# Belis0811/MaskUnet

Measured on AMD Instinct MI355X. Metric: 128x128 images/sec (fwd+bwd), higher is better.
Workload: dtype f16; 1 GPU; ADE20K-semantic shape 128x128, c_out=150, batch=64/GPU, 1-head MaskAttn-UNet fwd+bwd, train mode; global_batch=64, parallelism=dp1, mask_mode=fixed, loss=maskunet_amd.CrossEntropyLoss on module output, optimizer_in_step=False, hip_graph=False

## Files before the change

### maskunet_amd/csrc/elementwise.hip

```cpp
#include "common.h"
#include "../../include/maskunet_hip.h"

template <typename TS, typename TD>
__global__ __launch_bounds__(256) void transpose_kernel(const TS* __restrict__ src, long src_ld, TD* __restrict__ dst,
                                                        long dst_ld, int R, int C, int R_pad) {
    __shared__ float tile[64][65];
    const int b = blockIdx.z;
    const int r0 = blockIdx.y * 64, c0 = blockIdx.x * 64;
    const TS* s = src + (long)b * R * src_ld;
    TD* d = dst + (long)b * C * dst_ld;
    const int tx = threadIdx.x & 63, ty = threadIdx.x >> 6;
#pragma unroll 4
    for (int i = ty; i < 64; i += 4) {
        int r = r0 + i, c = c0 + tx;
        tile[i][tx] = (r < R && c < C) ? (float)s[(long)r * src_ld + c] : 0.f;
    }
    __syncthreads();
#pragma unroll 4
    for (int i = ty; i < 64; i += 4) {
        int c = c0 + i, r = r0 + tx;
        if (c < C && r < R_pad) d[(long)c * dst_ld + r] = (TD)tile[tx][i];
    }
}

// ... 63 lines not shown
    return mu_transpose_pad(src, src_dtype, src_ld, dst, dst_dtype, dst_ld, batch, R, C, R, stream);
}

template <typename T>
__global__ void prep_weight_kernel(const float* __restrict__ w, T* __restrict__ dst, int O, int I, int taps,
                                   int rows_pad, int cols_pad, int mode) {
    const long n = (long)taps * rows_pad * cols_pad;
    const long total = mode == 2 ? 2 * n : n;
    for (long idx = (long)blockIdx.x * blockDim.x + threadIdx.x; idx < total; idx += (long)gridDim.x * blockDim.x) {
        const bool second = idx >= n;
        const int m = mode == 2 ? (second ? 1 : 0) : mode;
        const long j = second ? idx - n : idx;
        const int rp = second ? cols_pad : rows_pad, cp = second ? rows_pad : cols_pad;
        int c = j % cp;
        int r = (j / cp) % rp;
        int t = j / ((long)cp * rp);
        float v = 0.f;
        if (m == 0) {
            if (r < O && c < I) v = w[((long)r * I + c) * taps + t];
        } else {
            if (r < I && c < O) v = w[((long)c * I + r) * taps + (taps - 1 - t)];
        }
        dst[idx] = (T)v;
    }
}

__global__ __launch_bounds__(256) void split_encode_kernel(const f32x4* src, uint4* dst, long n16);
__global__ __launch_bounds__(256) void split_encode_h4_kernel(const f32x4* src, uint4* dst, long n16, float scale);
__global__ __launch_bounds__(256) void encode_hl_rows_kernel(float* rows, long nrows, int len, float scale) {
    constexpr int MAXV = 8;
    const int nv = len / 4;
    for (long r = blockIdx.x; r < nrows; r += gridDim.x) {
        float* row = rows + r * len;
        f32x4 v[MAXV];
#pragma unroll
        for (int u = 0; u < MAXV; ++u)
            if (threadIdx.x + u * 256 < nv) v[u] = *reinterpret_cast<const f32x4*>(row + (threadIdx.x + u * 256) * 4) * scale;
        __syncthreads();
        h16* hrow = reinterpret_cast<h16*>(row);
#pragma unroll
        for (int u = 0; u < MAXV; ++u)
            if (threadIdx.x + u * 256 < nv) {
                const uint4 e = mu_ench4(v[u]);
                *reinterpret_cast<uint2*>(hrow + (threadIdx.x + u * 256) * 4) = make_uint2(e.z, e.w);
                *reinterpret_cast<uint2*>(hrow + len + (threadIdx.x + u * 256) * 4) = make_uint2(e.x, e.y);
            }
        __syncthreads();
    }
}

extern "C" int mu_prep_weight(const float* w_oihw, void* dst, int dtype, int O, int I, int taps, int rows_pad,
                              int cols_pad, int mode, void* stream) {
    if (!w_oihw || !dst || O <= 0 || I <= 0 || (taps != 1 && taps != 9)) return MU_ERR_ARG;
    if (mode < 0 || mode > 2) return MU_ERR_ARG;
    if (mode != 1 ? (rows_pad < O || cols_pad < I) : (rows_pad < I || cols_pad < O)) return MU_ERR_ARG;
    const bool enc = dtype == MU_F32X;
    const long n1 = (long)taps * rows_pad * cols_pad, n = n1 * (mode == 2 ? 2 : 1);
    const int len = mode == 2 ? rows_pad : cols_pad;
    if (enc && (rows_pad % 4 || cols_pad % 4)) return MU_ERR_SHAPE;
    if (enc && taps != 1 && mode != 0 && len > 8192) return MU_ERR_SHAPE;
    hipStream_t st = (hipStream_t)stream;
    const int rc = with_storage(enc ? MU_F32 : dtype, [&](auto tag) -> int {
        using T = decltype(tag);
        prep_weight_kernel<T><<<mu_grid(n, 256, 2048), 256, 0, st>>>(w_oihw, (T*)dst, O, I, taps, rows_pad, cols_pad, mode);
        return MU_OK;
    });
    if (rc) return rc;
    if (enc) {
        const float sh = (float)(1 << MU_XH_WSHIFT);
        float* d = (float*)dst;
        if (taps == 1) {
            split_encode_kernel<<<mu_grid(n / 4, 1024, 8192), 256, 0, st>>>((const f32x4*)d, (uint4*)d, n / 4);
        } else {
            if (mode != 1) split_encode_h4_kernel<<<mu_grid(n1 / 4, 1024, 8192), 256, 0, st>>>((const f32x4*)d, (uint4*)d, n1 / 4, sh);
            if (mode != 0) encode_hl_rows_kernel<<<mu_grid(n1 / len, 1, 4096), 256, 0, st>>>(mode == 2 ? d + n1 : d, n1 / len, len, sh);
        }
    }
    MU_CHECK_LAUNCH();
    return MU_OK;
}

#define MU_PREP_JOB_FIELDS 10
#define MU_PREP_MAX_JOBS 128
template <typename T, bool ENC = false>
__global__ __launch_bounds__(256) void prep_weights_multi_kernel(const long* __restrict__ jobs, int njobs, long ntiles, T* __restrict__ base) {
    constexpr int TS = 32, MAXT = 9, LD = TS * MAXT + 1;
    __shared__ long sj[MU_PREP_MAX_JOBS * MU_PREP_JOB_FIELDS];
    __shared__ float tile[TS * LD];
    for (int i = threadIdx.x; i < njobs * MU_PREP_JOB_FIELDS; i += blockDim.x) sj[i] = jobs[i];
    __syncthreads();
    for (long tl = blockIdx.x; tl < ntiles; tl += gridDim.x) {
        int lo = 0, hi = njobs - 1;
        while (lo < hi) {
            const int mid = (lo + hi + 1) >> 1;
            if (sj[mid * MU_PREP_JOB_FIELDS + 2] <= tl) lo = mid; else hi = mid - 1;
        }
        const long* J = sj + lo * MU_PREP_JOB_FIELDS;
        const float* w = reinterpret_cast<const float*>(J[0]);
        T* dst = base + J[1];
        const int O = (int)J[3], I = (int)J[4], taps = (int)J[5], rows_pad = (int)J[6], cols_pad = (int)J[7], mode = (int)J[8];
        const int tcols = cols_pad / TS;
        const int rel = (int)(tl - J[2]);
        const int o0 = (rel / tcols) * TS, i0 = (rel % tcols) * TS;
        const int run = TS * taps;
#pragma unroll 4
        for (int k = threadIdx.x; k < TS * run; k += 256) {
            const int ol = k / run, rem = k - ol * run;
            const int o = o0 + ol, i = i0 + rem / taps;
            tile[ol * LD + rem] = (o < O && i < I) ? w[((long)o * I + i0) * taps + rem] : 0.f;
        }
        __syncthreads();
        const long n = (long)taps * rows_pad * cols_pad;
        constexpr int VN = 16 / (int)sizeof(T), VPR = TS / VN;
        if (mode != 1)
            for (int k = threadIdx.x; k < taps * TS * VPR; k += 256) {
                const int iv = k % VPR, ol = (k / VPR) & 31, t = k / (VPR * TS);
                Vec16<T> v;
#pragma unroll
                for (int e = 0; e < VN; ++e) v.set(e, tile[ol * LD + (iv * VN + e) * taps + t]);
                T* q = dst + ((long)t * rows_pad + o0 + ol) * cols_pad + i0 + iv * VN;
                if constexpr (ENC) {
                    const f32x4 f = {v.get(0), v.get(1), v.get(2), v.get(3)};
                    *reinterpret_cast<uint4*>(q) = taps == 1 ? mu_enc4(f) : mu_ench4(f * (float)(1 << MU_XH_WSHIFT));
                } else v.store(q);
            }
        if (mode != 0) {
            T* d1 = mode == 2 ? dst + n : dst;
            for (int k = threadIdx.x; k < taps * TS * VPR; k += 256) {
                const int ov = k % VPR, il = (k / VPR) & 31, t = k / (VPR * TS);
                Vec16<T> v;
#pragma unroll
                for (int e = 0; e < VN; ++e) v.set(e, tile[(ov * VN + e) * LD + il * taps + t]);
                T* q = d1 + ((long)(taps - 1 - t) * cols_pad + i0 + il) * rows_pad + o0 + ov * VN;
                if constexpr (ENC) {
                    const f32x4 f = {v.get(0), v.get(1), v.get(2), v.get(3)};
                    if (taps == 1) *reinterpret_cast<uint4*>(q) = mu_enc4(f);
                    else {
                        const uint4 e4 = mu_ench4(f * (float)(1 << MU_XH_WSHIFT));
                        h16* hrow = reinterpret_cast<h16*>(d1 + ((long)(taps - 1 - t) * cols_pad + i0 + il) * rows_pad);
                        *reinterpret_cast<uint2*>(hrow + o0 + ov * VN) = make_uint2(e4.z, e4.w);
                        *reinterpret_cast<uint2*>(hrow + rows_pad + o0 + ov * VN) = make_uint2(e4.x, e4.y);
                    }
                } else v.store(q);
            }
        }
        __syncthreads();
    }
}

extern "C" int mu_prep_weights_multi(const void* jobs, int njobs, long ntiles, void* dst_base, int dtype, void* stream) {
    if (!jobs || !dst_base || njobs <= 0 || njobs > MU_PREP_MAX_JOBS || ntiles <= 0) return MU_ERR_ARG;
    const int grid = mu_grid(ntiles, 1, 4096);
    hipStream_t st = (hipStream_t)stream;
    if (dtype == MU_F32) prep_weights_multi_kernel<float><<<grid, 256, 0, st>>>((const long*)jobs, njobs, ntiles, (float*)dst_base);
    else if (dtype == MU_F32X) prep_weights_multi_kernel<float, true><<<grid, 256, 0, st>>>((const long*)jobs, njobs, ntiles, (float*)dst_base);
    else if (dtype == MU_F16) prep_weights_multi_kernel<h16><<<grid, 256, 0, st>>>((const long*)jobs, njobs, ntiles, (h16*)dst_base);
    else return MU_ERR_ARG;
    MU_CHECK_LAUNCH();
    return MU_OK;
}

template <typename TS, typename TD>
__global__ void cast_kernel(const TS* __restrict__ s, TD* __restrict__ d, long n) {
    for (long i = (long)blockIdx.x * blockDim.x + threadIdx.x; i < n; i += (long)gridDim.x * blockDim.x) d[i] = (TD)(float)s[i];
}
extern "C" int mu_cast(const void* src, int src_dtype, void* dst, int dst_dtype, long n, void* stream) {
    if (!src || !dst || n <= 0) return MU_ERR_ARG;
    hipStream_t st = (hipStream_t)stream;
    return with_storage2(src_dtype, dst_dtype, [&](auto stag, auto dtag) -> int {
        using TS = decltype(stag);
        using TD = decltype(dtag);
        cast_kernel<TS, TD><<<mu_grid(n, 256, 4096), 256, 0, st>>>((const TS*)src, (TD*)dst, n);
        MU_CHECK_LAUNCH();
        return MU_OK;
    });
}

__global__ __launch_bounds__(256) void split_encode_kernel(const f32x4* src, uint4* dst, long n16) {
    const long stride = (long)gridDim.x * 256;
    for (long i = (long)blockIdx.x * 256 + threadIdx.x; i < n16; i += 4 * stride) {
        f32x4 v[4];
#pragma unroll
        for (int u = 0; u < 4; ++u)
            if (i + u * stride < n16) v[u] = __builtin_nontemporal_load(src + i + u * stride);
#pragma unroll
        for (int u = 0; u < 4; ++u)
            if (i + u * stride < n16) dst[i + u * stride] = mu_enc4(v[u]);
    }
}
__global__ __launch_bounds__(256) void split_encode_h4_kernel(const f32x4* src, uint4* dst, long n16, float scale) {
    const long stride = (long)gridDim.x * 256;
    for (long i = (long)blockIdx.x * 256 + threadIdx.x; i < n16; i += 4 * stride) {
        f32x4 v[4];
#pragma unroll
        for (int u = 0; u < 4; ++u)
            if (i + u * stride < n16) v[u] = __builtin_nontemporal_load(src + i + u * stride);
#pragma unroll
        for (int u = 0; u < 4; ++u)
            if (i + u * stride < n16) dst[i + u * stride] = mu_ench4(v[u] * scale);
    }
}
__global__ __launch_bounds__(256) void split_encode_h4x_kernel(const f32x4* __restrict__ src, uint4* __restrict__ dst, uint2* __restrict__ dst16, long n16) {
    const long stride = (long)gridDim.x * 256;
    for (long i = (long)blockIdx.x * 256 + threadIdx.x; i < n16; i += 4 * stride) {
        f32x4 v[4];
#pragma unroll
        for (int u = 0; u < 4; ++u)
            if (i + u * stride < n16) v[u] = __builtin_nontemporal_load(src + i + u * stride);
#pragma unroll
        for (int u = 0; u < 4; ++u)
            if (i + u * stride < n16) {
                const uint4 e = mu_ench4(v[u]);
                dst[i + u * stride] = e;
                dst16[i + u * stride] = make_uint2(e.x, e.y);
            }
    }
}
extern "C" int mu_split_encode_h4x(const void* src, void* dst, void* dst16, long n_elems, void* stream) {
    if (!src || !dst || !dst16 || src == dst || n_elems <= 0 || n_elems % 4) return MU_ERR_ARG;
    const long n16 = n_elems / 4;
    split_encode_h4x_kernel<<<mu_grid(n16, 1024, 8192), 256, 0, (hipStream_t)stream>>>((const f32x4*)src, (uint4*)dst, (uint2*)dst16, n16);
    MU_CHECK_LAUNCH();
    return MU_OK;
}
extern "C" int mu_split_encode_h4(const void* src, void* dst, long n_elems, void* stream) {
    if (!src || !dst || n_elems <= 0 || n_elems % 4) return MU_ERR_ARG;
    const long n16 = n_elems / 4;
    split_encode_h4_kernel<<<mu_grid(n16, 1024, 8192), 256, 0, (hipStream_t)stream>>>((const f32x4*)src, (uint4*)dst, n16, 1.0f);
    MU_CHECK_LAUNCH();
// ... 842 lines not shown
```

### maskunet_amd/modules.py

```python
from __future__ import annotations

import torch
import torch.nn as nn

from . import ops
from ._lib import ACT_GELU, ACT_NONE, ACT_RELU

_DEFAULT_DTYPE = torch.float32


def set_default_compute_dtype(dtype):
    global _DEFAULT_DTYPE
    if dtype not in (torch.float32, torch.float16):
        raise TypeError("compute dtype must be torch.float32 or torch.float16")
    _DEFAULT_DTYPE = dtype


class _HipModule(nn.Module):
    def __init__(self):
        super().__init__()
        self.compute_dtype = _DEFAULT_DTYPE

    def set_compute_dtype(self, dtype):
        if dtype not in (torch.float32, torch.float16):
# ... 166 lines not shown

    def forward_nhwc(self, x, skip_x, cx=None, cs=None, skip_link=None):
        link = ops.grad_link(x, skip_x)
        x = ops.upcat(x, skip_x, cx, cs, link, skip_link)
        return _conv_blocks(x, [self.conv[0], self.conv[1]], self.conv[2], link)

    def forward(self, x, skip_x):
        self._check_device(x)
        y = self.forward_nhwc(ops.to_nhwc(x, self.compute_dtype), ops.to_nhwc(skip_x, self.compute_dtype), x.shape[1], skip_x.shape[1])
        return ops.to_nchw(y, self.out_channels, x.dtype)


class _Head(nn.Sequential):
    """Conv2d 1x1 (bias) -> BatchNorm2d -> ReLU container with the reference's Sequential indices."""


def _head_1x1_bn_relu(seq, x):
    if ops.eval_fusable(seq[1]):
        return ops.conv_bn_act_eval(x, seq[0].weight, seq[0].bias, seq[1], ACT_RELU)
    y = ops.conv(x, seq[0].weight, seq[0].bias)
    return ops.bn_act(y, seq[1], ACT_RELU)


class UNet(_HipModule):

    def __init__(self, c_in=3, c_out=3, embed_dim=None, *, hw=128):
        super().__init__()
        self.c_out = c_out
        self.initial_conv = ConvBlock(c_in, 64)
        self.downsample1 = DownSample(64, 128)
        self.self_attention1 = Mask2FormerAttention(128, 128)
        self.downsample2 = DownSample(128, 256)
        self.self_attention2 = Mask2FormerAttention(256, 256)
        self.downsample3 = DownSample(256, 256)
        self.self_attention3 = Mask2FormerAttention(256, 256)

        self.bottom1 = ConvBlock(256, 512)
        self.bottom2 = ConvBlock(512, 512)
        self.bottom3 = ConvBlock(512, 256)

        self.dropout = nn.Dropout(0.3)

        self.upsample1 = UpSample(512, 128)
        self.self_attention4 = Mask2FormerAttention(128, 128)
        self.upsample2 = UpSample(256, 64)
        self.self_attention5 = Mask2FormerAttention(64, 64)
        self.upsample3 = UpSample(128, 64)
        self.self_attention6 = Mask2FormerAttention(64, 64)
        self.norm = nn.LayerNorm([64, hw, hw])
        self.final_layer = nn.Sequential(nn.Conv2d(64, c_out, kernel_size=1), nn.BatchNorm2d(c_out), nn.ReLU())
        self.three_head = embed_dim is not None
        if self.three_head:
            self.boundary_head = nn.Sequential(
                nn.Conv2d(c_out, 32, kernel_size=3, padding=1), nn.BatchNorm2d(32), nn.ReLU(), nn.Conv2d(32, 1, kernel_size=1))
            self.embedding_head = nn.Sequential(nn.Conv2d(64, embed_dim, kernel_size=1), nn.BatchNorm2d(embed_dim), nn.ReLU())
            self.embed_dim = embed_dim
        self.dropout_masks = None

    def attention_blocks(self):
        return [getattr(self, f"self_attention{i}") for i in range(1, 7)]

    def set_keep_masks(self, keeps):
        for blk, k in zip(self.attention_blocks(), keeps):
            blk.set_keep_mask(k)

    def set_mask_mode(self, mode):
        if mode not in ("fixed", "resample"):
            raise ValueError("mask_mode must be 'fixed' or 'resample'")
        for blk in self.attention_blocks():
            blk.mask_mode = mode

    def _drop(self, x, i):
        m = None if self.dropout_masks is None else self.dropout_masks[i]
        return ops.dropout(x, self.dropout.p, self.training, m)

    def forward_nhwc(self, x):
        if not (torch.is_grad_enabled() and self.training and ops.MULTI_PREP):
            return self._forward_nhwc(x)
        ws = self.__dict__.get("_conv_ws")
        if ws is None:
            ws = self.__dict__["_conv_ws"] = ([m for m in self.modules() if isinstance(m, nn.Conv2d)], {})
        weights = [m.weight for m in ws[0]]
        first = self.initial_conv.conv_block[0].weight
        ops.prep_conv_weights(ws[1], weights, x.dtype, fwd_only=() if x.requires_grad else (first,))
        try:
            return self._forward_nhwc(x)
        finally:
            for w in weights:
                w._mu_step = None

    def _forward_nhwc(self, x):
        x1 = self.initial_conv.forward_nhwc(x)
        l1 = ops.grad_link(x1)
        x2 = self.downsample1.forward_nhwc(x1, skip_link=l1)
        x2 = self.self_attention1.forward_nhwc(x2)
        l2 = ops.grad_link(x2)
        x3 = self.downsample2.forward_nhwc(x2, skip_link=l2)
        x3 = self.self_attention2.forward_nhwc(x3)
        l3 = ops.grad_link(x3)
        x4 = self.downsample3.forward_nhwc(x3, skip_link=l3)
        x4 = ops.cut_point(self.self_attention3.forward_nhwc(x4))

        x4 = _conv_blocks(x4, [self.bottom1, self.bottom2, self.bottom3])

        y = self.upsample1.forward_nhwc(x4, x3, skip_link=l3)
        y = self._drop(y, 0)
        y = self.self_attention4.forward_nhwc(y)
        y = self.upsample2.forward_nhwc(y, x2, skip_link=l2)
        y = self._drop(y, 1)
        y = self.self_attention5.forward_nhwc(y)
        y = self.upsample3.forward_nhwc(y, x1, skip_link=l1)
        B, H, W, _ = y.shape
        y = self.self_attention6.forward_nhwc(y, scramble=False)
        if tuple(self.norm.normalized_shape) != (64, H, W):
            raise RuntimeError(f"Given normalized_shape={list(self.norm.normalized_shape)}, expected input with shape "
                               f"[*, 64, {H}, {W}]")
        y = ops.ln_sample(y.view(B, -1), self.norm.weight, self.norm.bias, self.norm.eps)
        y = ops.to_nhwc(y.view(B, 64, H, W), self.compute_dtype)
        sem = _head_1x1_bn_relu(self.final_layer, y)
        if not self.three_head:
            return (sem,)
        emb = _head_1x1_bn_relu(self.embedding_head, y)
        bh = self.boundary_head
        if ops.eval_fusable(bh[1]):
            b = ops.conv_bn_act_eval(sem, bh[0].weight, bh[0].bias, bh[1], ACT_RELU)
        else:
            b = ops.conv(sem, bh[0].weight, bh[0].bias)
            b = ops.bn_act(b, bh[1], ACT_RELU)
        b = ops.conv(b, bh[3].weight, bh[3].bias)
        return sem, b, emb

    def logits_nhwc(self, x):
        self._check_device(x)
        return self.forward_nhwc(ops.to_nhwc(x, self.compute_dtype))[0]

    def forward_u8(self, images_u8_hwc, bgr=False, resample="cv2", check=False):
        if resample == "pil":
            from . import images as _images
            packed = _images.pack_images(images_u8_hwc)
            self._check_device(packed.data)
            H, W = int(self.norm.normalized_shape[1]), int(self.norm.normalized_shape[2])
            x, valid = _images.resize_pil_to_nhwc(packed, (H, W), self.compute_dtype, bgr=bgr)
            if check and not bool(valid.all()):
                raise RuntimeError(f"maskunet_amd: the Pillow resize refused images {(valid == 0).nonzero().flatten().tolist()} (size outside "
                                   "the contract: taller than 100 widths)")
            return self._finish(self.forward_nhwc(x))
        if resample != "cv2":
            raise ValueError(f'resample must be "cv2" or "pil", got {resample!r}')
        self._check_device(images_u8_hwc)
        H, W = int(self.norm.normalized_shape[1]), int(self.norm.normalized_shape[2])
        if tuple(images_u8_hwc.shape[1:3]) == (H, W) and not bgr:
            x = ops.u8_hwc_to_nhwc(images_u8_hwc, self.compute_dtype)
        else:
            x = ops.resize_u8_to_nhwc(images_u8_hwc, (W, H), self.compute_dtype, bgr=bgr)
        return self._finish(self.forward_nhwc(x))

    def forward(self, x):
        self._check_device(x)
        return self._finish(self.forward_nhwc(ops.to_nhwc(x, self.compute_dtype)))

    def _finish(self, outs):
        sem = ops.to_nchw(outs[0], self.c_out, torch.float32)
        if not self.three_head:
            return sem
        return sem, ops.to_nchw(outs[1], 1, torch.float32), ops.to_nchw(outs[2], self.embed_dim, torch.float32)


class InstanceUNet(UNet):

    def __init__(self, c_in=3, c_out=3, embed_dim=16, *, hw=128):
        super().__init__(c_in, c_out, embed_dim, hw=hw)

# ... 19 lines not shown
```

### maskunet_amd/ops.py

```python
from __future__ import annotations

import math
import os
from types import SimpleNamespace
from typing import NamedTuple

import torch
import torch.nn.functional as F
from torch.autograd.function import once_differentiable

from . import _lib
from ._lib import ACT_GELU, ACT_NONE, ACT_RELU, call, dt, mdt, ptr, stream, workspace


def pad32(c: int) -> int:
    return (c + 31) // 32 * 32


def _pad_vec(v, n, fill):
    v = v.detach().float()
    if v.numel() == n:
        return v.contiguous()
    return F.pad(v, (0, n - v.numel()), value=fill)

# ... 147 lines not shown
    B, H, W, C = img_u8.shape
    y = torch.empty((B, H, W, pad32(C)), dtype=dtype, device=img_u8.device)
    call("mu_u8_to_nhwc", ptr(img_u8), ptr(y), B * H * W, C, pad32(C), dt(y), stream())
    return y


def resize_u8_to_nhwc(img_u8, size, dtype, bgr=False, return_u8=False):
    img_u8 = img_u8.contiguous()
    if img_u8.dtype != torch.uint8 or img_u8.dim() != 4 or img_u8.shape[-1] > 4:
        raise RuntimeError("resize_u8_to_nhwc expects a uint8 [B,H,W,C<=4] tensor")
    B, Hs, Ws, C = img_u8.shape
    Wd, Hd = int(size[0]), int(size[1])
    y = torch.empty((B, Hd, Wd, pad32(C)), dtype=dtype, device=img_u8.device)
    u8 = torch.empty((B, Hd, Wd, C), dtype=torch.uint8, device=img_u8.device) if return_u8 else None
    call("mu_resize_u8_nhwc", ptr(img_u8), B, Hs, Ws, C, int(bool(bgr)), ptr(y), ptr(u8), Hd, Wd, pad32(C), dt(y), stream())
    return (y, u8) if return_u8 else y


def resize_labels_u8(mask_u8, size):
    mask_u8 = mask_u8.contiguous()
    if mask_u8.dtype != torch.uint8 or mask_u8.dim() != 3:
        raise RuntimeError("resize_labels_u8 expects a uint8 [B,H,W] tensor")
    B, Hs, Ws = mask_u8.shape
    Wd, Hd = int(size[0]), int(size[1])
    out = torch.empty((B, Hd, Wd), dtype=torch.int64, device=mask_u8.device)
    call("mu_resize_nearest_u8", ptr(mask_u8), B, Hs, Ws, ptr(out), Hd, Wd, stream())
    return out


def to_nchw(x, C, out_dtype=torch.float32):
    y = _ToNCHW.apply(x, C, out_dtype)
    y._mu_nhwc = (x, C, y._version)
    return y


PREP_CACHE = os.environ.get("MU_PREP_CACHE", "1") != "0"


def _cache_ok():
    return PREP_CACHE and not torch.is_grad_enabled()


def _prep_cached(w, key, make, ok, extra_tag=()):
    if not ok or torch.cuda.is_current_stream_capturing():
        return make()
    cache = getattr(w, "_mu_prep", None)
    if cache is None:
        cache = {}
        try:
            w._mu_prep = cache
        except Exception:
            return make()
    tag = (w._version, w.data_ptr()) + tuple(extra_tag)
    hit = cache.get(key)
    if hit is not None and hit[0] == tag:
        return hit[1]
    out = make()
    cache[key] = (tag, out)
    return out


def _prep_weight(w, dtype, rows_pad, cols_pad, mode, cache_ok=False):
    if cache_ok and isinstance(w, torch.nn.Parameter):
        return _prep_cached(w, (dtype, mdt(dtype), rows_pad, cols_pad, mode), lambda: _prep_weight_raw(w, dtype, rows_pad, cols_pad, mode), True)
    return _prep_weight_raw(w, dtype, rows_pad, cols_pad, mode)


def _prep_weight_raw(w, dtype, rows_pad, cols_pad, mode):
    O, I = w.shape[0], w.shape[1]
    taps = w.shape[2] * w.shape[3] if w.dim() == 4 else 1
    n = taps * rows_pad * cols_pad
    dst = torch.empty((2 * n if mode == 2 else n,), dtype=dtype, device=w.device)
    wf = w.detach().float().contiguous()
    call("mu_prep_weight", ptr(wf), ptr(dst), mdt(dtype), O, I, taps, rows_pad, cols_pad, mode, stream())
    if mode == 2:
        return dst[:n].view(taps, rows_pad, cols_pad), dst[n:].view(taps, cols_pad, rows_pad)
    return dst.view(taps, rows_pad, cols_pad)


MULTI_PREP = os.environ.get("MU_MULTI_PREP", "1") != "0"
MULTI_PREP_MAX_JOBS = 128


def prep_conv_weights(holder, weights, dtype, fwd_only=()):
    if not MULTI_PREP or not weights:
        return
    dev = weights[0].device
    if dev.type != "cuda" or any(w.dtype != torch.float32 or not w.is_contiguous() or w.dim() != 4 for w in weights):
        return
    if len(weights) > MULTI_PREP_MAX_JOBS or any(w.shape[2] * w.shape[3] not in (1, 9) for w in weights):
        return
    only = {id(w) for w in fwd_only}
    key = (dtype, mdt(dtype), tuple((w.data_ptr(), tuple(w.shape)) for w in weights), tuple(id(w) in only for w in weights))
    plans = holder.setdefault("plans", {})
    plan = plans.get(key)
    capturing = torch.cuda.is_current_stream_capturing()
    if plan is not None and capturing:
        holder.setdefault("pinned", {})[key] = plan
    if plan is None:
        if capturing:
            return
        rows, metas, off, chunk = [], [], 0, 0
        for w in weights:
            O, I, taps = w.shape[0], w.shape[1], w.shape[2] * w.shape[3]
            rp, cp = pad32(O), pad32(I)
            n = taps * rp * cp
            mode = 0 if id(w) in only else 2
            total = n if mode == 0 else 2 * n
            rows.append([w.data_ptr(), off, chunk, O, I, taps, rp, cp, mode, 0])
            metas.append((off, n, taps, rp, cp, mode))
            off += total
            chunk += (rp // 32) * (cp // 32)
        plan = plans[key] = (key, torch.tensor(rows, dtype=torch.int64, device=dev), metas, off, chunk)
        pinned = holder.get("pinned", {})
        for old in [k for k in plans if k != key and k not in pinned][:max(0, len(plans) - len(pinned) - 8)]:
            del plans[old]
    _, table, metas, total, nchunks = plan
    dst = torch.empty(total, dtype=dtype, device=dev)
    call("mu_prep_weights_multi", ptr(table), len(weights), nchunks, ptr(dst), mdt(dtype), stream())
    tag = (dtype, mdt(dtype))
    for w, (off, n, taps, rp, cp, mode) in zip(weights, metas):
        fwd = dst[off:off + n].view(taps, rp, cp)
        wd = dst[off + n:off + 2 * n].view(taps, cp, rp) if mode == 2 else None
        w._mu_step = (w._version, w.data_ptr(), tag, fwd, wd)


def _take_step_prep(w, dtype, taps, rows_pad, cols_pad, need_dgrad):
    pre = getattr(w, "_mu_step", None)
    if pre is None:
        return None
    w._mu_step = None
    if pre[0] != w._version or pre[1] != w.data_ptr() or pre[2] != (dtype, mdt(dtype)) or tuple(pre[3].shape) != (taps, rows_pad, cols_pad):
        return None
    if need_dgrad and pre[4] is None:
        return None
    return pre[3], pre[4]


def _conv_raw(x, wprep, bias_p, Cout_p, taps, want_stats=False):
    B, H, W, Cin_p = x.shape
    y = torch.empty((B, H, W, Cout_p), dtype=x.dtype, device=x.device)
    part = None
    if want_stats and (rows := _lib.load().mu_conv_stats_rows(B, H, W, Cin_p, Cout_p, taps, mdt(x))) > 0:
        part = torch.empty((rows, Cout_p, 2), dtype=torch.float32, device=x.device)
        call("mu_conv_fwd_stats", ptr(x), ptr(wprep), ptr(bias_p), ptr(y), B, H, W, Cin_p, Cout_p, taps, Cin_p, Cout_p, mdt(x),
             ptr(part), stream())
    else:
        call("mu_conv_fwd", ptr(x), ptr(wprep), ptr(bias_p), ptr(y), B, H, W, Cin_p, Cout_p, taps, Cin_p, Cout_p, mdt(x), stream())
    return (y, part) if want_stats else y


CUT_HOOK = None


def cut_point(t):
    if CUT_HOOK is not None and t.requires_grad:
        t.register_hook(CUT_HOOK)
    return t


GRAD_ARENA = None
GRAD_HANDED = set()


def grad_out(param, shape, device):
    a = GRAD_ARENA
    if a is not None and param is not None and getattr(param, "grad", None) is None:
        v = a.get(id(param))
        if v is not None and v.device == device and v.numel() == math.prod(shape) and v.data_ptr() not in GRAD_HANDED:
            GRAD_HANDED.add(v.data_ptr())
            return v.view(shape)
    return torch.empty(shape, dtype=torch.float32, device=device)


def _wgrad_h1(x16, dyh, w_shape, param=None):
    B, H, W, Cin_p = x16.shape
    O, I = w_shape[0], w_shape[1]
    Cout_p = dyh.h.shape[-1]
    gw = grad_out(param, tuple(w_shape), x16.device)
    ws = workspace(_lib.load().mu_conv_wgrad_workspace_bytes(B, H, W, Cin_p, Cout_p, 9), x16.device)
    call("mu_conv_wgrad_h1", ptr(x16), ptr(dyh.h), ptr(dyh.scale), ptr(gw), B, H, W, Cin_p, Cout_p, I, O, Cin_p, Cout_p, ptr(ws), ws.numel(),
         stream())
    return gw


def _wgrad_raw(x, gy, w_shape, taps, gy_enc=False, x_enc=False, param=None):
    B, H, W, Cin_p = x.shape
    O, I = w_shape[0], w_shape[1]
    code = mdt(x)
    if code == _lib.MU_F32X and taps == 9:
        if I > 3 or gy_enc or x_enc:
            raise RuntimeError("conv weight gradient: an fp32x 3x3 layer takes the fp16 rounding of its input (mu_conv_wgrad_h1)")
        code = _lib.MU_F32
    if code == _lib.MU_F32X:
        if not x_enc:
            x = _enc(x)
        if not gy_enc:
            gy = _enc(gy)
    Cout_p = gy.shape[-1]
    gw = grad_out(param, tuple(w_shape), x.device)
    ws = workspace(_lib.load().mu_conv_wgrad_workspace_bytes(B, H, W, Cin_p, Cout_p, taps), x.device)
    call("mu_conv_wgrad", ptr(x), ptr(gy), ptr(gw), B, H, W, Cin_p, Cout_p, taps, I, O, Cin_p, Cout_p, ptr(ws), ws.numel(), code, stream())
    return gw


def _wgrad_bias_raw(x, gy, w_shape, taps, param=None):
    B, H, W, Cin_p = x.shape
# ... 519 lines not shown

class _LNSample(torch.autograd.Function):

    @staticmethod
    def forward(ctx, x, w, b, eps):
        x = x.contiguous()
        B = x.shape[0]
        L = x.numel() // B
        wf, bf = w.detach().float().contiguous().view(-1), b.detach().float().contiguous().view(-1)
        y = torch.empty_like(x)
        mean = torch.empty(B, dtype=torch.float32, device=x.device)
        rstd = torch.empty_like(mean)
        ws = workspace(_lib.load().mu_ln_sample_workspace_bytes(B), x.device)
        call("mu_ln_sample_fwd", ptr(x), ptr(wf), ptr(bf), ptr(y), ptr(mean), ptr(rstd), B, L, float(eps), ptr(ws), ws.numel(),
             dt(x), stream())
        ctx.save_for_backward(x, wf, mean, rstd)
        ctx.wshape = tuple(w.shape)
        ctx.wparam, ctx.bparam = w, b
        return y

    @staticmethod
    @once_differentiable
    def backward(ctx, gy):
        x, wf, mean, rstd = ctx.saved_tensors
        gy = gy.contiguous()
        B = x.shape[0]
        L = x.numel() // B
        dx = torch.empty_like(x)
        dw = grad_out(ctx.wparam, (L,), x.device)
        db = grad_out(ctx.bparam, (L,), x.device)
        ws = workspace(_lib.load().mu_ln_sample_workspace_bytes(B), x.device)
        call("mu_ln_sample_bwd", ptr(x), ptr(gy), ptr(wf), ptr(mean), ptr(rstd), ptr(dx), ptr(dw), ptr(db), B, L, ptr(ws),
             ws.numel(), dt(x), stream())
        return dx, dw.view(ctx.wshape), db.view(ctx.wshape), None


def ln_sample(x, w, b, eps):
    return _LNSample.apply(x, w, b, eps)


def _transpose_tokens(src, R, C):
    B = src.shape[0]
    dst = torch.empty((B, C, R), dtype=src.dtype, device=src.device)
    call("mu_transpose", ptr(src), dt(src), C, ptr(dst), dt(dst), R, B, R, C, stream())
    return dst


def _pad_param(t, C):
    return F.pad(t.detach().float(), [p for n in reversed(t.shape) for p in (0, C - n)])


def _refuse_padded_scramble(scramble, cv, C):
    if scramble and cv != C:
        raise RuntimeError("mask_attention: the re-viewed (scrambled) output needs an unpadded channel count")


def _attn_entry(name, cv, head, tail):
    if cv == head[-1]:
        call(name, *head, *tail)
    else:
        call(name + "_padded", *head, cv, *tail)


def _attn_grads(gx, gw, gb, dg, db, C, cv, n_rest):
    return (gx, gw[:cv, :cv], gb[:cv], gw[C:C + cv, :cv], gb[C:C + cv], gw[2 * C:2 * C + cv, :cv], gb[2 * C:2 * C + cv],
            dg[:cv], db[:cv]) + (None,) * n_rest


class _MaskAttention(torch.autograd.Function):

    @staticmethod
    def forward(ctx, x, wq, bq, wk, bk, wv, bv, lnw, lnb, kidx, kcnt, eps, scramble, cache_ok=False, kidx_perm=False):
        x = x.contiguous()
        B, H, W, C = x.shape
        N = H * W
        cv = wq.shape[0]
        ctx.cv = cv
        if cv != C:
            _refuse_padded_scramble(scramble, cv, C)
            wq, wk, wv, bq, bk, bv, lnw, lnb = (_pad_param(t, C) for t in (wq, wk, wv, bq, bk, bv, lnw, lnb))
            cache_ok = False

        def make_qkv():
            wbuf = torch.empty((6 * C * C,), dtype=x.dtype, device=x.device)
            bqkv_ = torch.empty((3 * C,), dtype=torch.float32, device=x.device)
            src = [t.detach() if t.dtype == torch.float32 and t.is_contiguous() else t.detach().float().contiguous()
                   for t in (wq, wk, wv, bq, bk, bv)]
            call("mu_prep_qkv", *[ptr(t) for t in src], ptr(wbuf), ptr(bqkv_), dt(x), C, stream())
            _enc_(wbuf)
            return bqkv_, (wbuf[:3 * C * C].view(1, 3 * C, C), wbuf[3 * C * C:].view(1, C, 3 * C))

        if cache_ok and isinstance(wq, torch.nn.Parameter):
            vers = tuple((t._version, t.data_ptr()) for t in (wk, wv, bq, bk, bv))
            bqkv, (wprep, wd_) = _prep_cached(wq, ("qkv", x.dtype, mdt(x)), make_qkv, True, extra_tag=vers)
        else:
            bqkv, (wprep, wd_) = make_qkv()
        ctx.wd = wd_ if ctx.needs_input_grad[0] else None
        xe = _enc(x)
        if _is_x(x) and QKV_ENCODED and (3 * C) % 64 == 0:
            qkv = torch.empty((B, H, W, 3 * C), dtype=x.dtype, device=x.device)
            call("mu_conv1x1_fwd_enc_h", ptr(xe), ptr(wprep), ptr(bqkv), ptr(qkv), B * N, C, 3 * C, C, 3 * C, stream())
        else:
            qkv = _enc_h_(_conv_raw(xe, wprep, bqkv, 3 * C, 1))
        out = torch.empty((B, N, C), dtype=x.dtype, device=x.device)
        oattn = torch.empty_like(out)
        lse2 = torch.empty((B, N), dtype=torch.float32, device=x.device)
        mean, rstd = torch.empty_like(lse2), torch.empty_like(lse2)
        g, b_ = lnw.detach().float().contiguous(), lnb.detach().float().contiguous()
        _attn_entry("mu_attn_fwd", cv, (ptr(qkv), ptr(x), ptr(kidx), ptr(kcnt), ptr(g), ptr(b_), ptr(out), ptr(oattn), ptr(lse2), ptr(mean),
                                        ptr(rstd), B, N, C), (kidx.shape[1], float(eps), mdt(x), stream()))
        ctx.save_for_backward(x, qkv, oattn, lse2, mean, rstd, g, kidx, kcnt, xe)
        ctx.is_x = _is_x(x)
        ctx.scramble, ctx.dims, ctx.kidx_perm = scramble, (B, H, W, C), bool(kidx_perm) and kidx.shape[1] == N
        if scramble:
            return _transpose_tokens(out.view(B, C, N), C, N).view(B, H, W, C)
        return out

    @staticmethod
    @once_differentiable
    def backward(ctx, gout):
        x, qkv, oattn, lse2, mean, rstd, g, kidx, kcnt, xe = ctx.saved_tensors
        B, H, W, C = ctx.dims
        N = H * W
        gout = gout.contiguous()
        _same_mode(ctx.is_x, gout)
        if ctx.scramble:
            gout = _transpose_tokens(gout.view(B, N, C), N, C)
        dY = torch.empty((B, N, C), dtype=x.dtype, device=x.device)
        dqkv = torch.empty((B, N, 3 * C), dtype=x.dtype, device=x.device)
        delta = torch.empty((B, N), dtype=torch.float32, device=x.device)
        dg = torch.empty(C, dtype=torch.float32, device=x.device)
        db = torch.empty_like(dg)
        ws = workspace(_lib.load().mu_attn_bwd_workspace_bytes(B, N, C), x.device)
        perm = 8 if ctx.kidx_perm else 0
        enc_dqkv = ctx.is_x and DQKV_ENCODED
        if enc_dqkv:
            perm |= 16
        for phase in (1, 2, 4):
            _attn_entry("mu_attn_bwd_phases", ctx.cv, (ptr(qkv), ptr(x), ptr(oattn), ptr(gout), ptr(kidx), ptr(kcnt), ptr(lse2), ptr(mean),
                                                       ptr(rstd), ptr(g), ptr(dY), ptr(delta), ptr(dqkv), ptr(dg), ptr(db), B, N, C),
                        (kidx.shape[1], ptr(ws), ws.numel(), mdt(x), phase | perm, stream()))
        dqkv4 = dqkv.view(B, H, W, 3 * C)
        dqkv_e = dqkv4 if enc_dqkv else _enc(dqkv4)
        gx = None
        if ctx.needs_input_grad[0]:
            wd = ctx.wd
            if ATTN_FUSED_ADD and _lib.load().mu_conv1x1_add_supported(3 * C, C, mdt(x)):
                gx = torch.empty((B, H, W, C), dtype=x.dtype, device=x.device)
                call("mu_conv1x1_fwd_add", ptr(dqkv_e), ptr(wd), ptr(dY), ptr(gx), B * N, 3 * C, C, 3 * C, C, mdt(x), stream())
            else:
                gx = _conv_raw(dqkv_e, wd, None, C, 1)
                call("mu_add", ptr(gx), ptr(dY), ptr(gx), gx.numel(), dt(gx), stream())
        both = None if enc_dqkv else _wgrad_bias_raw(x, dqkv4, (3 * C, C, 1, 1), 1)
        if both is not None:
            gw, gb = both[0].view(3 * C, C), both[1]
        else:
            gw = _wgrad_raw(xe, dqkv_e, (3 * C, C, 1, 1), 1, gy_enc=True, x_enc=ctx.is_x).view(3 * C, C)
            gb = _colsum(dqkv4, 3 * C, encoded=enc_dqkv)
        return _attn_grads(gx, gw, gb, dg, db, C, ctx.cv, 6)


ATTN_FUSED_ADD = os.environ.get("MU_ATTN_FUSED_ADD", "1") != "0"
QKV_ENCODED = os.environ.get("MU_QKV_ENCODED", "1") != "0"
DQKV_ENCODED = os.environ.get("MU_DQKV_ENCODED", "1") != "0"


# ... 136 lines not shown
```

Before: 2306 images/sec.

## Fold QKV weight prep into batched weight-prep kernel and software-pipeline tile loads

```diff
diff --git a/maskunet_amd/csrc/elementwise.hip b/maskunet_amd/csrc/elementwise.hip
--- a/maskunet_amd/csrc/elementwise.hip
+++ b/maskunet_amd/csrc/elementwise.hip
@@ -169,69 +169,192 @@
 
 #define MU_PREP_JOB_FIELDS 10
 #define MU_PREP_MAX_JOBS 128
+#define MU_PREP_PLANE (32 * 32 + 2)
+struct PrepTile {
+    const float* w;
+    long dst_off;
+    int O, I, taps, rows_pad, cols_pad, mode, row0, o0, i0;
+};
+__device__ __forceinline__ PrepTile prep_tile_of(const long* __restrict__ jobs, const long* first, int njobs, long tl) {
+    int lo = 0, hi = njobs - 1;
+    while (lo < hi) {
+        const int mid = (lo + hi + 1) >> 1;
+        if (first[mid] <= tl) lo = mid; else hi = mid - 1;
+    }
+    const long* J = jobs + lo * MU_PREP_JOB_FIELDS;
+    PrepTile p;
+    p.w = reinterpret_cast<const float*>(J[0]);
+    p.dst_off = J[1];
+    p.O = (int)J[3], p.I = (int)J[4], p.taps = (int)J[5], p.rows_pad = (int)J[6], p.cols_pad = (int)J[7], p.mode = (int)J[8];
+    p.row0 = p.mode == 3 ? (int)J[9] : 0;
+    if (p.mode >= 3) p.taps = 1;
+    const int tcols = p.cols_pad >= 32 ? p.cols_pad / 32 : 1;
+    const int rel = (int)(tl - first[lo]);
+    p.o0 = (rel / tcols) * 32, p.i0 = (rel % tcols) * 32;
+    return p;
+}
+template <int VN>
+__device__ __forceinline__ int prep_pos(int x, int y) {
+    constexpr int VPR = 32 / VN, NP = VN / 2;
+    return ((((x % VN) >> 1) ^ ((y >> 1) & (NP - 1))) * (2 * VPR)) + (x / VN) * 2 + (x & 1);
+}
+typedef const __attribute__((address_space(1))) float* PrepGlobal;
+__device__ __forceinline__ int prep_tid() {
+    int t = threadIdx.x;
+    asm volatile("" : "+v"(t));
+    return t;
+}
+__device__ __forceinline__ bool prep_fast(const PrepTile& p) {
+    return (p.taps == 9 || p.taps == 1) && p.mode <= 3 && p.I % 4 == 0 && (reinterpret_cast<size_t>(p.w) & 15) == 0;
+}
+template <int TAPS>
+__device__ __forceinline__ void prep_load(const PrepTile& p, f32x4* v) {
+    constexpr int RUN4 = 8 * TAPS, NV = RUN4 * 32 / 256;
+    const int ncol = (p.I - p.i0 < 32 ? p.I - p.i0 : 32) * TAPS;
+    const PrepGlobal w = (PrepGlobal)p.w;
+    const int tid = prep_tid();
+#pragma unroll
+    for (int u = 0; u < NV; ++u) {
+        const int k = tid + 256 * u, ol = k / RUN4, c = (k % RUN4) * 4;
+        const int o = p.o0 + ol;
+        f32x4 r = {0.f, 0.f, 0.f, 0.f};
+        if (o < p.O && c < ncol) r = *reinterpret_cast<const __attribute__((address_space(1))) f32x4*>(w + ((long)o * p.I + p.i0) * TAPS + c);
+        v[u] = r;
+    }
+}
+template <typename T, bool ENC, int TAPS, bool TR>
+__device__ __forceinline__ void prep_store(const PrepTile& p, const f32x4* v, float* lds, T* __restrict__ base) {
+    constexpr int RUN4 = 8 * TAPS, NV = RUN4 * 32 / 256;
+    constexpr int VN = 16 / (int)sizeof(T), VPR = 32 / VN;
+    const int tid = prep_tid();
+#pragma unroll
+    for (int u = 0; u < NV; ++u) {
+        const int k = tid + 256 * u, ol = k / RUN4, c = (k % RUN4) * 4;
+#pragma unroll
+        for (int e = 0; e < 4; ++e) {
+            const int i = (c + e) / TAPS, t = (c + e) % TAPS;
+            lds[t * MU_PREP_PLANE + (TR ? i * 32 + prep_pos<VN>(ol, i) : ol * 32 + prep_pos<VN>(i, ol))] = v[u][e];
+        }
+    }
+    __syncthreads();
+    const long n = (long)TAPS * p.rows_pad * p.cols_pad;
+    T* dst = base + p.dst_off + (TR && p.mode != 1 ? n : 0);
+    for (int k = tid; k < TAPS * 32 * VPR; k += 256) {
+        const int g = k % VPR, r = (k / VPR) & 31, t = k / (VPR * 32);
+        Vec16<T> x;
+#pragma unroll
+        for (int j = 0; j < VN / 2; ++j) {
+            const float2 f = *reinterpret_cast<const float2*>(lds + t * MU_PREP_PLANE + r * 32 + prep_pos<VN>(g * VN + 2 * j, r));
+            x.set(2 * j, f.x);
+            x.set(2 * j + 1, f.y);
+        }
+        const long row = TR ? (long)(TAPS - 1 - t) * p.cols_pad + p.i0 + r : (long)t * p.rows_pad + p.row0 + p.o0 + r;
+        const int ld = TR ? p.rows_pad : p.cols_pad, col = (TR ? p.row0 + p.o0 : p.i0) + g * VN;
+        T* q = dst + row * ld + col;
+        if constexpr (ENC) {
+            const f32x4 f = {x.get(0), x.get(1), x.get(2), x.get(3)};
+            if (TAPS == 1) *reinterpret_cast<uint4*>(q) = mu_enc4(f);
+            else if (!TR) *reinterpret_cast<uint4*>(q) = mu_ench4(f * (float)(1 << MU_XH_WSHIFT));
+            else {
+                const uint4 e4 = mu_ench4(f * (float)(1 << MU_XH_WSHIFT));
+                h16* hrow = reinterpret_cast<h16*>(dst + row * ld);
+                *reinterpret_cast<uint2*>(hrow + col) = make_uint2(e4.z, e4.w);
+                *reinterpret_cast<uint2*>(hrow + ld + col) = make_uint2(e4.x, e4.y);
+            }
+        } else x.store(q);
+    }
+    __syncthreads();
+}
+template <typename T, bool ENC, int TAPS>
+__device__ __forceinline__ void prep_tile_fast(const PrepTile& p, const f32x4* v, float* lds, T* __restrict__ base) {
+    if (p.mode != 1) prep_store<T, ENC, TAPS, false>(p, v, lds, base);
+    if (p.mode != 0) prep_store<T, ENC, TAPS, true>(p, v, lds, base);
+}
+
+template <typename T, bool ENC>
+__device__ void prep_tile_generic(const PrepTile& p, float* tile, T* __restrict__ base) {
+    constexpr int TS = 32, MAXT = 9, LD = TS * MAXT + 1;
+    const float* w = p.w;
+    T* dst = base + p.dst_off;
+    const int O = p.O, I = p.I, taps = p.taps, rows_pad = p.rows_pad, cols_pad = p.cols_pad, mode = p.mode == 3 ? 2 : p.mode;
+    const int o0 = p.o0, i0 = p.i0;
+    const int run = TS * taps;
+#pragma unroll 4
+    for (int k = threadIdx.x; k < TS * run; k += 256) {
+        const int ol = k / run, rem = k - ol * run;
+        const int o = o0 + ol, i = i0 + rem / taps;
+        tile[ol * LD + rem] = (o < O && i < I) ? w[((long)o * I + i0) * taps + rem] : 0.f;
+    }
+    __syncthreads();
+    const long n = (long)taps * rows_pad * cols_pad;
+    constexpr int VN = 16 / (int)sizeof(T), VPR = TS / VN;
+    if (mode != 1)
+        for (int k = threadIdx.x; k < taps * TS * VPR; k += 256) {
+            const int iv = k % VPR, ol = (k / VPR) & 31, t = k / (VPR * TS);
+            Vec16<T> v;
+#pragma unroll
+            for (int e = 0; e < VN; ++e) v.set(e, tile[ol * LD + (iv * VN + e) * taps + t]);
+            T* q = dst + ((long)t * rows_pad + o0 + ol) * cols_pad + i0 + iv * VN;
+            if constexpr (ENC) {
+                const f32x4 f = {v.get(0), v.get(1), v.get(2), v.get(3)};
+                *reinterpret_cast<uint4*>(q) = taps == 1 ? mu_enc4(f) : mu_ench4(f * (float)(1 << MU_XH_WSHIFT));
+            } else v.store(q);
+        }
+    if (mode != 0) {
+        T* d1 = mode == 2 ? dst + n : dst;
+        for (int k = threadIdx.x; k < taps * TS * VPR; k += 256) {
+            const int ov = k % VPR, il = (k / VPR) & 31, t = k / (VPR * TS);
+            Vec16<T> v;
+#pragma unroll
+            for (int e = 0; e < VN; ++e) v.set(e, tile[(ov * VN + e) * LD + il * taps + t]);
+            T* q = d1 + ((long)(taps - 1 - t) * cols_pad + i0 + il) * rows_pad + o0 + ov * VN;
+            if constexpr (ENC) {
+                const f32x4 f = {v.get(0), v.get(1), v.get(2), v.get(3)};
+                if (taps == 1) *reinterpret_cast<uint4*>(q) = mu_enc4(f);
+                else {
+                    const uint4 e4 = mu_ench4(f * (float)(1 << MU_XH_WSHIFT));
+                    h16* hrow = reinterpret_cast<h16*>(d1 + ((long)(taps - 1 - t) * cols_pad + i0 + il) * rows_pad);
+                    *reinterpret_cast<uint2*>(hrow + o0 + ov * VN) = make_uint2(e4.z, e4.w);
+                    *reinterpret_cast<uint2*>(hrow + rows_pad + o0 + ov * VN) = make_uint2(e4.x, e4.y);
+                }
+            } else v.store(q);
+        }
+    }
+    __syncthreads();
+}
+
 template <typename T, bool ENC = false>
-__global__ __launch_bounds__(256) void prep_weights_multi_kernel(const long* __restrict__ jobs, int njobs, long ntiles, T* __restrict__ base) {
-    constexpr int TS = 32, MAXT = 9, LD = TS * MAXT + 1;
-    __shared__ long sj[MU_PREP_MAX_JOBS * MU_PREP_JOB_FIELDS];
-    __shared__ float tile[TS * LD];
-    for (int i = threadIdx.x; i < njobs * MU_PREP_JOB_FIELDS; i += blockDim.x) sj[i] = jobs[i];
+__global__ __launch_bounds__(256, 4) void prep_weights_multi_kernel(const long* __restrict__ jobs, int njobs, long ntiles, T* __restrict__ base) {
+    __shared__ long first[MU_PREP_MAX_JOBS];
+    __shared__ __attribute__((aligned(16))) float lds[32 * (32 * 9 + 1)];
+    static_assert(9 * MU_PREP_PLANE <= 32 * (32 * 9 + 1), "LDS tile");
+    for (int i = threadIdx.x; i < njobs; i += blockDim.x) first[i] = jobs[i * MU_PREP_JOB_FIELDS + 2];
     __syncthreads();
-    for (long tl = blockIdx.x; tl < ntiles; tl += gridDim.x) {
-        int lo = 0, hi = njobs - 1;
-        while (lo < hi) {
-            const int mid = (lo + hi + 1) >> 1;
-            if (sj[mid * MU_PREP_JOB_FIELDS + 2] <= tl) lo = mid; else hi = mid - 1;
-        }
-        const long* J = sj + lo * MU_PREP_JOB_FIELDS;
-        const float* w = reinterpret_cast<const float*>(J[0]);
-        T* dst = base + J[1];
-        const int O = (int)J[3], I = (int)J[4], taps = (int)J[5], rows_pad = (int)J[6], cols_pad = (int)J[7], mode = (int)J[8];
-        const int tcols = cols_pad / TS;
-        const int rel = (int)(tl - J[2]);
-        const int o0 = (rel / tcols) * TS, i0 = (rel % tcols) * TS;
-        const int run = TS * taps;
-#pragma unroll 4
-        for (int k = threadIdx.x; k < TS * run; k += 256) {
-            const int ol = k / run, rem = k - ol * run;
-            const int o = o0 + ol, i = i0 + rem / taps;
-            tile[ol * LD + rem] = (o < O && i < I) ? w[((long)o * I + i0) * taps + rem] : 0.f;
-        }
-        __syncthreads();
-        const long n = (long)taps * rows_pad * cols_pad;
-        constexpr int VN = 16 / (int)sizeof(T), VPR = TS / VN;
-        if (mode != 1)
-            for (int k = threadIdx.x; k < taps * TS * VPR; k += 256) {
-                const int iv = k % VPR, ol = (k / VPR) & 31, t = k / (VPR * TS);
-                Vec16<T> v;
-#pragma unroll
-                for (int e = 0; e < VN; ++e) v.set(e, tile[ol * LD + (iv * VN + e) * taps + t]);
-                T* q = dst + ((long)t * rows_pad + o0 + ol) * cols_pad + i0 + iv * VN;
-                if constexpr (ENC) {
-                    const f32x4 f = {v.get(0), v.get(1), v.get(2), v.get(3)};
-                    *reinterpret_cast<uint4*>(q) = taps == 1 ? mu_enc4(f) : mu_ench4(f * (float)(1 << MU_XH_WSHIFT));
-                } else v.store(q);
+    PrepTile cur, nxt;
+    f32x4 vc[9], vn[9];
+    bool have = false;
+    for (long tl = (long)blockIdx.x - gridDim.x; tl < ntiles; tl += gridDim.x) {
+        const bool more = tl + gridDim.x < ntiles;
+        if (more) {
+            nxt = prep_tile_of(jobs, first, njobs, tl + gridDim.x);
+            if (prep_fast(nxt)) {
+                if (nxt.taps == 9) prep_load<9>(nxt, vn);
+                else prep_load<1>(nxt, vn);
             }
-        if (mode != 0) {
-            T* d1 = mode == 2 ? dst + n : dst;
-            for (int k = threadIdx.x; k < taps * TS * VPR; k += 256) {
-                const int ov = k % VPR, il = (k / VPR) & 31, t = k / (VPR * TS);
-                Vec16<T> v;
-#pragma unroll
-                for (int e = 0; e < VN; ++e) v.set(e, tile[(ov * VN + e) * LD + il * taps + t]);
-                T* q = d1 + ((long)(taps - 1 - t) * cols_pad + i0 + il) * rows_pad + o0 + ov * VN;
-                if constexpr (ENC) {
-                    const f32x4 f = {v.get(0), v.get(1), v.get(2), v.get(3)};
-                    if (taps == 1) *reinterpret_cast<uint4*>(q) = mu_enc4(f);
-                    else {
-                        const uint4 e4 = mu_ench4(f * (float)(1 << MU_XH_WSHIFT));
-                        h16* hrow = reinterpret_cast<h16*>(d1 + ((long)(taps - 1 - t) * cols_pad + i0 + il) * rows_pad);
-                        *reinterpret_cast<uint2*>(hrow + o0 + ov * VN) = make_uint2(e4.z, e4.w);
-                        *reinterpret_cast<uint2*>(hrow + rows_pad + o0 + ov * VN) = make_uint2(e4.x, e4.y);
-                    }
-                } else v.store(q);
-            }
-        }
-        __syncthreads();
+        }
+        if (have) {
+            if (cur.mode == 4) {
+                float* b = reinterpret_cast<float*>(base + cur.dst_off);
+                for (int k = threadIdx.x; k < cur.O; k += 256) b[k] = ((PrepGlobal)cur.w)[k];
+            } else if (prep_fast(cur)) {
+                if (cur.taps == 9) prep_tile_fast<T, ENC, 9>(cur, vc, lds, base);
+                else prep_tile_fast<T, ENC, 1>(cur, vc, lds, base);
+            } else if (cur.taps >= 1 && cur.taps <= 9 && cur.mode <= 2) prep_tile_generic<T, ENC>(cur, lds, base);
+        }
+        cur = nxt;
+        have = more;
+#pragma unroll
+        for (int u = 0; u < 9; ++u) vc[u] = vn[u];
     }
 }
 
diff --git a/maskunet_amd/modules.py b/maskunet_amd/modules.py
--- a/maskunet_amd/modules.py
+++ b/maskunet_amd/modules.py
@@ -272,12 +272,16 @@
             ws = self.__dict__["_conv_ws"] = ([m for m in self.modules() if isinstance(m, nn.Conv2d)], {})
         weights = [m.weight for m in ws[0]]
         first = self.initial_conv.conv_block[0].weight
-        ops.prep_conv_weights(ws[1], weights, x.dtype, fwd_only=() if x.requires_grad else (first,))
+        qkv = [tuple(t for lin in (a.query, a.key, a.value) for t in (lin.weight, lin.bias)) for a in self.attention_blocks()
+               if a.query.weight.shape[0] == ops.attn_width(a.query.weight.shape[0]) and a.query.weight.shape[0] <= ops.ATTN_WIDTHS[-1]]
+        ops.prep_conv_weights(ws[1], weights, x.dtype, fwd_only=() if x.requires_grad else (first,), qkv=qkv)
         try:
             return self._forward_nhwc(x)
         finally:
             for w in weights:
                 w._mu_step = None
+            for b in qkv:
+                b[0]._mu_step_qkv = None
 
     def _forward_nhwc(self, x):
         x1 = self.initial_conv.forward_nhwc(x)
diff --git a/maskunet_amd/ops.py b/maskunet_amd/ops.py
--- a/maskunet_amd/ops.py
+++ b/maskunet_amd/ops.py
@@ -253,7 +253,13 @@
 MULTI_PREP_MAX_JOBS = 128
 
 
-def prep_conv_weights(holder, weights, dtype, fwd_only=()):
+def _qkv_rides(block, dev):
+    C = block[0].shape[0]
+    return (C % 32 == 0 and all(t.device == dev and t.dtype == torch.float32 and t.is_contiguous() and t.data_ptr() % 16 == 0 for t in block)
+            and all(tuple(t.shape) == (C, C) for t in block[0::2]) and all(tuple(t.shape) == (C,) for t in block[1::2]))
+
+
+def prep_conv_weights(holder, weights, dtype, fwd_only=(), qkv=()):
     if not MULTI_PREP or not weights:
         return
     dev = weights[0].device
@@ -261,8 +267,12 @@
         return
     if len(weights) > MULTI_PREP_MAX_JOBS or any(w.shape[2] * w.shape[3] not in (1, 9) for w in weights):
         return
+    qkv = [tuple(b) for b in qkv if _qkv_rides(tuple(b), dev)]
+    if len(weights) + 6 * len(qkv) > MULTI_PREP_MAX_JOBS:
+        qkv = []
     only = {id(w) for w in fwd_only}
-    key = (dtype, mdt(dtype), tuple((w.data_ptr(), tuple(w.shape)) for w in weights), tuple(id(w) in only for w in weights))
+    key = (dtype, mdt(dtype), tuple((w.data_ptr(), tuple(w.shape)) for w in weights), tuple(id(w) in only for w in weights),
+           tuple((t.data_ptr(), b[0].shape[0]) for b in qkv for t in b))
     plans = holder.setdefault("plans", {})
     plan = plans.get(key)
     capturing = torch.cuda.is_current_stream_capturing()
@@ -282,18 +292,46 @@
             metas.append((off, n, taps, rp, cp, mode))
             off += total
             chunk += (rp // 32) * (cp // 32)
+        esz = torch.empty((), dtype=dtype).element_size()
+        qmetas = []
+        for wq, bq, wk, bk, wv, bv in qkv:
+            C = wq.shape[0]
+            boff = off + 6 * C * C
+            for j, (w, b) in enumerate(((wq, bq), (wk, bk), (wv, bv))):
+                rows.append([w.data_ptr(), off, chunk, C, C, 1, 3 * C, C, 3, j * C])
+                chunk += (C // 32) * (C // 32)
+                rows.append([b.data_ptr(), boff + j * C * 4 // esz, chunk, C, 1, 1, 32, 32, 4, 0])
+                chunk += 1
+            qmetas.append((off, boff, C))
+            off = boff + 3 * C * 4 // esz
+        metas = (metas, qmetas)
         plan = plans[key] = (key, torch.tensor(rows, dtype=torch.int64, device=dev), metas, off, chunk)
         pinned = holder.get("pinned", {})
         for old in [k for k in plans if k != key and k not in pinned][:max(0, len(plans) - len(pinned) - 8)]:
             del plans[old]
-    _, table, metas, total, nchunks = plan
+    _, table, (metas, qmetas), total, nchunks = plan
     dst = torch.empty(total, dtype=dtype, device=dev)
-    call("mu_prep_weights_multi", ptr(table), len(weights), nchunks, ptr(dst), mdt(dtype), stream())
+    call("mu_prep_weights_multi", ptr(table), table.shape[0], nchunks, ptr(dst), mdt(dtype), stream())
     tag = (dtype, mdt(dtype))
     for w, (off, n, taps, rp, cp, mode) in zip(weights, metas):
         fwd = dst[off:off + n].view(taps, rp, cp)
         wd = dst[off + n:off + 2 * n].view(taps, cp, rp) if mode == 2 else None
         w._mu_step = (w._version, w.data_ptr(), tag, fwd, wd)
+    for block, (off, boff, C) in zip(qkv, qmetas):
+        n = 3 * C * C
+        bias = dst[boff:boff + 3 * C * 4 // dst.element_size()].view(torch.float32)
+        block[0]._mu_step_qkv = (tuple((t._version, t.data_ptr()) for t in block), tag, C, bias,
+                                 (dst[off:off + n].view(1, 3 * C, C), dst[off + n:off + 2 * n].view(1, C, 3 * C)))
+
+
+def _take_step_qkv(block, dtype, C):
+    pre = getattr(block[0], "_mu_step_qkv", None)
+    if pre is None:
+        return None
+    block[0]._mu_step_qkv = None
+    if pre[0] != tuple((t._version, t.data_ptr()) for t in block) or pre[1] != (dtype, mdt(dtype)) or pre[2] != C:
+        return None
+    return pre[3], pre[4]
 
 
 def _take_step_prep(w, dtype, taps, rows_pad, cols_pad, need_dgrad):
@@ -979,6 +1017,9 @@
             cache_ok = False
 
         def make_qkv():
+            pre = _take_step_qkv((wq, bq, wk, bk, wv, bv), x.dtype, C)
+            if pre is not None:
+                return pre
             wbuf = torch.empty((6 * C * C,), dtype=x.dtype, device=x.device)
             bqkv_ = torch.empty((3 * C,), dtype=torch.float32, device=x.device)
             src = [t.detach() if t.dtype == torch.float32 and t.is_contiguous() else t.detach().float().contiguous()
```

After: 2314 images/sec (median of 6 runs). Within noise of the previous version (+0.4%).
